# thu-ml/tianshou

Hardware: AMD Instinct MI355X
Metric: PPO learn() update-steps/sec (minibatch 65536, preprocessing incl.) + GAE transitions/sec; cpu_baseline / rocm_eager_baseline are PORTS of the reference path (oracle/), kind=port (higher is better)
Workload: dtype f32; 1 GPU; C2 PPO MuJoCo-shape rollout (BASELINE configs[1]): ONE rollout of 512 envs x 2048 steps = 2^20 transitions, minibatch 65536, obs 17, act 6, MLP[64,64] actor-critic, repeat 10, recompute_advantage off; parallelism=dp1, exchange=none

## Files before the change

include/tsengine.h:

```cpp
#ifndef TSENGINE_H
#define TSENGINE_H

#include <stddef.h>
#include <stdint.h>

#ifdef __cplusplus
extern "C" {
#endif

#define TS_OK 0
#define TS_ERR_INVALID_ARG (-1)
#define TS_ERR_SHAPE (-2)
#define TS_ERR_HIP (-3)
#define TS_ERR_UNSUPPORTED (-4)
#define TS_ERR_WORKSPACE (-5)

typedef void* ts_stream_t;
typedef struct ts_workspace ts_workspace;

const char* ts_version(void);
const char* ts_last_error(void);

int ts_workspace_create(ts_workspace** out, int device, size_t max_bytes);
int ts_workspace_destroy(ts_workspace* ws);
// ... 3 lines not shown
#define TS_KIND_PPO_STEP 0
#define TS_KIND_PPO_REDUCE 1
#define TS_KIND_PPO_ADAM 2
#define TS_KIND_PPO_INFER 3
#define TS_KIND_GAE_MAPS 4
#define TS_KIND_GAE_APPLY 5
#define TS_KIND_CONV_FWD 6
#define TS_KIND_CONV_WGRAD 7
#define TS_KIND_CONV_DGRAD 8
#define TS_N_KINDS 9
int ts_profile_begin(ts_workspace* ws);
int ts_profile_end(ts_workspace* ws, double* h_ms_by_kind, int64_t* h_count_by_kind, int n_kinds);


int64_t ts_gae_num_tiles(int64_t n);
int ts_gae_scan(ts_workspace* ws, const float* v_s, const float* v_s_next, const void* rew,
                int rew_dtype, const uint8_t* terminated, const uint8_t* truncated,
                const int64_t* cut_pos, int64_t n_cut, const int64_t* d_n_cut, int64_t n,
                double gamma, double gae_lambda, double v_scale, double ret_div, float* adv_out,
                float* returns_out, double* adv64, double* ret64, double* ret_partials,
                ts_stream_t stream);

int ts_gae_check(ts_workspace* ws, int* h_error_out, ts_stream_t stream);

int ts_isin_positions(const int64_t* indices, int64_t n, const int64_t* unfinished,
                      int64_t n_unfinished, int64_t* cut_pos_out, int64_t capacity,
                      int64_t* n_cut_out, ts_stream_t stream);

int ts_nstep_return(const double* rew_B, const uint8_t* end_flag_B, const float* target_q_IA,
                    const int64_t* stacked_indices_NI, int64_t I, int64_t A, int64_t n_step,
                    int64_t B, double gamma, float* out, double* out64, ts_stream_t stream);

int ts_nstep_indices(const int64_t* indices, int64_t I, int64_t n_step, const int64_t* offset,
                     int64_t E, const uint8_t* done, const int64_t* last_index,
                     const int64_t* lengths, int64_t* after_out, int64_t* stacked_out,
                     ts_stream_t stream);

int ts_nstep_return_fused(const int64_t* indices, int64_t I, int64_t n_step,
                          const int64_t* offset, int64_t E, const uint8_t* done,
                          const uint8_t* terminated, const int64_t* last_index,
                          const int64_t* lengths, const double* rew_B, const float* target_q_IA,
                          int64_t A, double gamma, float* out, double* out64,
                          ts_stream_t stream);

int ts_nstep_coefficients(const int64_t* indices, int64_t I, int64_t n_step, const int64_t* offset, int64_t E,
                          const uint8_t* done_B, const uint8_t* terminated_B, const int64_t* last_index,
// ... 89 lines not shown
    int32_t optimizer;
    int32_t rms_centered;
    double weight_decay;
    double rms_alpha;
    double rms_momentum;
    double max_action;
} ts_ppo_hparams;
#define TS_OPT_ADAM 0
#define TS_OPT_RMSPROP 1

int ts_ppo_infer(ts_workspace* ws, const float* params, int64_t obs_dim, int64_t act_dim, const float* obs,
                 const float* act, int64_t n, float* v_out, float* logp_out,
                 ts_stream_t stream);
int ts_ppo_infer_bounded(ts_workspace* ws, const float* params, int64_t obs_dim, int64_t act_dim, double max_action,
                         const float* obs, const float* act, int64_t n, float* v_out, float* logp_out, float* mu_out,
                         ts_stream_t stream);

int ts_ppo_update(ts_workspace* ws, float* params, float* adam_m, float* adam_v,
                  int64_t adam_step0, int64_t obs_dim, int64_t act_dim, const float* obs,
                  const float* act, const float* adv, const float* returns,
                  const float* logp_old, const float* v_s, int64_t n, const int64_t* perm,
                  const int64_t* h_mb_offset, int64_t n_steps, const ts_ppo_hparams* hp,
                  float* losses_out, float* grads_out, ts_stream_t stream);

int64_t ts_ppo_record_width(int64_t obs_dim, int64_t act_dim);
int ts_ppo_pack_batch(const float* obs, const float* act, const float* adv, const float* returns,
                      const float* logp_old, const float* v_s, int64_t n, int64_t obs_dim,
                      int64_t act_dim, float* rec_out, ts_stream_t stream);

int ts_ppo_grad(ts_workspace* ws, const float* params, int64_t obs_dim, int64_t act_dim,
                const float* rec, int64_t n, const int64_t* perm_rows, int64_t n_rows,
                int64_t global_batch, const float* adv_stats, const ts_ppo_hparams* hp,
                float* grad_out, float* loss_parts_out, ts_stream_t stream);
int ts_ppo_apply(ts_workspace* ws, float* params, float* adam_m, float* adam_v, int64_t adam_step, int64_t obs_dim,
                 int64_t act_dim, const float* grad, const ts_ppo_hparams* hp, ts_stream_t stream);
int ts_ppo_invalidate_image(ts_workspace* ws);

int ts_ppo_step_plan(int64_t obs_dim, int64_t act_dim, int64_t n_rows, int32_t nets, int32_t* variant_out,
                     int32_t* grid_out, int32_t* slabs_out);


int ts_polyak_update(float* tgt, const float* src, int64_t n, double tau, ts_stream_t stream);

int ts_adam_step(ts_workspace* ws, float* params, float* adam_m, float* adam_v, const float* grad, int64_t n,
                 int64_t step, double lr, double beta1, double beta2, double eps, double max_grad_norm,
                 ts_stream_t stream);
// ... 492 lines not shown
```

tianshou_amd/_lib.py:

```python
from __future__ import annotations

import ctypes as C
import os
import re

_PKG = os.path.dirname(os.path.abspath(__file__))
LIB_PATH = os.environ.get("TS_LIB_PATH") or os.path.join(_PKG, "lib", "libtsengine.so")
HEADER_PATH = os.path.join(os.path.dirname(_PKG), "include", "tsengine.h")

TS_OK = 0
TS_ERR_INVALID_ARG = -1
TS_ERR_SHAPE = -2
TS_ERR_HIP = -3
TS_ERR_UNSUPPORTED = -4
TS_ERR_WORKSPACE = -5


class EngineError(RuntimeError):

    def __init__(self, code: int, msg: str):
        super().__init__(f"libtsengine error {code}: {msg}")
        self.code = code


# ... 130 lines not shown
    @property
    def handle(self) -> C.c_void_p:
        return self._h

    profiling = False

    def profile_begin(self) -> None:
        check(load().ts_profile_begin(self._h))
        self.profiling = True

    def profile_end(self) -> dict[str, tuple[float, int]]:
        n = len(KERNEL_KINDS)
        ms = (C.c_double * n)()
        cnt = (C.c_int64 * n)()
        check(load().ts_profile_end(self._h, ms, cnt, C.c_int(n)))
        self.profiling = False
        return {k: (float(ms[i]), int(cnt[i])) for i, k in enumerate(KERNEL_KINDS)}

    def gae_check(self) -> int:
        err = C.c_int(0)
        check(load().ts_gae_check(self._h, C.byref(err), current_stream()))
        return int(err.value)

    def close(self) -> None:
        if self._h:
            load().ts_workspace_destroy(self._h)
            self._h = C.c_void_p(0)

    def __del__(self):
        try:
            self.close()
        except Exception:
            pass


_default_ws: dict[tuple[int, int], Workspace] = {}


def default_workspace(device_index: int) -> Workspace:
    import torch

    try:
        stream = int(_raw_stream(device_index))
    except Exception:
        stream = 0
    key = (device_index, stream)
# ... 22 lines not shown
```

tianshou_amd/csrc/ts_common.h:

```cpp
#pragma once
#include <hip/hip_runtime.h>

#include <atomic>
#include <cstdarg>
#include <cstdint>
#include <cstdio>

#include "../../include/tsengine.h"

namespace ts {

char* err_buf();
int fail(int code, const char* fmt, ...);

#define TS_HIP_CHECK(expr)                                                                 \
    do {                                                                                   \
        hipError_t _e = (expr);                                                            \
        if (_e != hipSuccess)                                                              \
            return ts::fail(TS_ERR_HIP, "%s failed: %s (%s:%d)", #expr, hipGetErrorString(_e), \
                            __FILE__, __LINE__);                                           \
    } while (0)

#define TS_LAUNCH_CHECK()                                                                  \
    do {                                                                                   \
// ... 26 lines not shown
    unsigned long long gae_ticket_base[8];
    unsigned int gae_epoch;
    int profiling;
    hipEvent_t* ev;
    int* ev_kind;
    int ev_cap, ev_n;
    void* ppo_image;
    size_t ppo_image_bytes;
    const float* ppo_image_params;
    int ppo_image_key;
    void* conv_scratch[2];
    size_t conv_scratch_bytes[2];
    void* dg_tables;
    long long dg_key[16][16];
    int dg_next[2];
    hipStream_t side;
    hipStream_t side2;
    hipEvent_t side_ev[16];
    int side_ready;
    hipEvent_t td_ev;
    int td_ev_ready;
    void* learn_graphs;
    void (*learn_graphs_free)(void*);
};

namespace ts {
int ws_reserve(ts_workspace* ws, size_t bytes);
int ws_winner(ts_workspace* ws, int64_t bound, hipStream_t stream, int32_t** out);

int side_stream(ts_workspace* ws, hipStream_t main, hipStream_t* out);
int stream_wait(ts_workspace* ws, hipStream_t from, hipStream_t to, int slot);
int side_streams(ts_workspace* ws, hipStream_t main, hipStream_t* a, hipStream_t* b);
int record_td(ts_workspace* ws, hipStream_t s);
void adam_step_scalars(int64_t step, double lr, double beta1, double beta2, float out[2]);
int adam_step_dev(hipStream_t s, float* params, float* m, float* v, const float* grad, int64_t n, const float* step_dev,
                  double beta1, double beta2, double eps, double max_grad_norm, float* norm_scratch);
int uniform_fill_f64(double* out, int64_t n, uint64_t seed, uint64_t counter, const uint64_t* counter_dev, hipStream_t s);

struct DynLds {
    std::atomic<int> granted[16] = {};
    int allow(const void* fn, size_t bytes) {
        int dev = 0;
        if (hipGetDevice(&dev) != hipSuccess || dev < 0) dev = 0;
        std::atomic<int>& g = granted[dev & 15];
        if ((int)bytes <= g.load(std::memory_order_acquire)) return TS_OK;
        hipError_t e = hipFuncSetAttribute(fn, hipFuncAttributeMaxDynamicSharedMemorySize, (int)bytes);
// ... 55 lines not shown
```

tianshou_amd/csrc/ts_core.hip:

```cpp
#include <cstdlib>
#include <cstring>

#include "ts_common.h"

namespace ts {

char* err_buf() {
    static thread_local char buf[512] = {0};
    return buf;
}

int fail(int code, const char* fmt, ...) {
    va_list ap;
    va_start(ap, fmt);
    vsnprintf(err_buf(), 512, fmt, ap);
    va_end(ap);
    return code;
}

int ws_reserve(ts_workspace* ws, size_t bytes) {
    if (!ws) return fail(TS_ERR_WORKSPACE, "workspace is NULL");
    if (bytes <= ws->bytes) return TS_OK;
    if (ws->max_bytes && bytes > ws->max_bytes)
        return fail(TS_ERR_WORKSPACE, "workspace needs %zu bytes, limit is %zu", bytes, ws->max_bytes);
// ... 146 lines not shown
    return TS_OK;
}

int ts_workspace_side_stream(ts_workspace* ws, int which, ts_stream_t* stream_out) {
    TS_REQUIRE(ws != nullptr && stream_out != nullptr, TS_ERR_WORKSPACE, "ts_workspace_side_stream: NULL argument");
    TS_REQUIRE(which == 0 || which == 1, TS_ERR_INVALID_ARG, "ts_workspace_side_stream: which = 0 or 1");
    if (int rc = ts::side_create(ws)) return rc;
    *stream_out = reinterpret_cast<ts_stream_t>(which == 0 ? ws->side : ws->side2);
    return TS_OK;
}

int ts_workspace_destroy(ts_workspace* ws) {
    if (!ws) return TS_OK;
    if (ws->learn_graphs && ws->learn_graphs_free) { (void)hipSetDevice(ws->device); ws->learn_graphs_free(ws->learn_graphs); }
    if (ws->side_ready) {
        (void)hipSetDevice(ws->device);
        (void)hipStreamSynchronize(ws->side);
        for (int i = 0; i < 16; ++i) (void)hipEventDestroy(ws->side_ev[i]);
        (void)hipStreamSynchronize(ws->side2);
        (void)hipStreamDestroy(ws->side);
        (void)hipStreamDestroy(ws->side2);
    }
    if (ws->td_ev_ready) { (void)hipSetDevice(ws->device); (void)hipEventDestroy(ws->td_ev); }
    if (ws->ppo_image) { (void)hipSetDevice(ws->device); (void)hipDeviceSynchronize(); (void)hipFree(ws->ppo_image); }
    for (int k = 0; k < 2; ++k)
        if (ws->conv_scratch[k]) { (void)hipSetDevice(ws->device); (void)hipDeviceSynchronize(); (void)hipFree(ws->conv_scratch[k]); }
    if (ws->dg_tables) { (void)hipSetDevice(ws->device); (void)hipDeviceSynchronize(); (void)hipFree(ws->dg_tables); }
    if (ws->base || ws->winner || ws->ev || ws->gae_sync) {
        (void)hipSetDevice(ws->device);
        (void)hipDeviceSynchronize();
        if (ws->gae_sync) (void)hipFree(ws->gae_sync);
        if (ws->base) (void)hipFree(ws->base);
        if (ws->winner) (void)hipFree(ws->winner);
        if (ws->ev) {
            for (int i = 0; i < 2 * ws->ev_cap; ++i) (void)hipEventDestroy(ws->ev[i]);
            free(ws->ev);
            free(ws->ev_kind);
        }
    }
    free(ws);
    return TS_OK;
}

}
```

tianshou_amd/csrc/ts_ppo.hip:

```cpp
#include <cstdlib>

#include "ts_common.h"

namespace {

using f32x16 = __attribute__((ext_vector_type(16))) float;
using f32x4 = __attribute__((ext_vector_type(4))) float;

constexpr int HID = 64;
constexpr int W2_PITCH = 68;
constexpr int W2_SIZE = HID * W2_PITCH;
constexpr int ACT_PAD = 8;
constexpr int TILE_PITCH = 36;
constexpr int TILE_SIZE = 32 * TILE_PITCH;
constexpr int STEP_THREADS = 256;
constexpr int STEP_WAVES = STEP_THREADS / 64;
constexpr int N_EXTRA = 2;

__device__ __forceinline__ int featF(int r, int h) { return (r & 3) + 8 * (r >> 2) + 4 * h; }

__device__ __forceinline__ f32x16 mfma32(float a, float b, f32x16 c) {
    return __builtin_amdgcn_mfma_f32_32x32x2f32(a, b, c, 0, 0, 0);
}

// ... 1128 lines not shown
                                                       const float* __restrict__ ret,
                                                       const float* __restrict__ logp_old,
                                                       const float* __restrict__ v_old, int64_t n,
                                                       int obs_dim, int act_dim, int rec_w,
                                                       float* __restrict__ rec) {
    const int64_t total = n * rec_w;
    const int64_t stride = (int64_t)gridDim.x * blockDim.x;
    for (int64_t t = (int64_t)blockIdx.x * blockDim.x + threadIdx.x; t < total; t += stride) {
        const int64_t row = t / rec_w;
        const int c = (int)(t - row * rec_w);
        float v = 0.f;
        if (c < obs_dim) v = obs[row * obs_dim + c];
        else if (c < obs_dim + act_dim) v = act[row * act_dim + (c - obs_dim)];
        else if (c == obs_dim + act_dim) v = adv[row];
        else if (c == obs_dim + act_dim + 1) v = ret[row];
        else if (c == obs_dim + act_dim + 2) v = logp_old[row];
        else if (c == obs_dim + act_dim + 3) v = v_old[row];
        rec[t] = v;
    }
}

__global__ __launch_bounds__(1024) void ppo_adv_stats_kernel(const float* __restrict__ adv,
                                                             const int64_t* __restrict__ perm,
                                                             const int64_t* __restrict__ mb_offset,
                                                             float* __restrict__ out) {
    __shared__ double r1[16], r2[16];
    const int64_t lo = mb_offset[blockIdx.x], hi = mb_offset[blockIdx.x + 1];
    double s1 = 0.0, s2 = 0.0;
    for (int64_t k = lo + threadIdx.x; k < hi; k += 1024) {
        const double v = (double)adv[perm ? perm[k] : k];
        s1 += v;
        s2 += v * v;
    }
#pragma unroll
    for (int off = 32; off > 0; off >>= 1) {
        s1 += __shfl_down(s1, off, 64);
        s2 += __shfl_down(s2, off, 64);
    }
    if ((threadIdx.x & 63) == 0) { r1[threadIdx.x >> 6] = s1; r2[threadIdx.x >> 6] = s2; }
    __syncthreads();
    if (threadIdx.x == 0) {
        double t1 = 0.0, t2 = 0.0;
        for (int w = 0; w < 16; ++w) { t1 += r1[w]; t2 += r2[w]; }
        const double n = (double)(hi - lo);
        const double mean = t1 / n;
        const double var = (t2 - n * mean * mean) / (n - 1.0);
        out[2 * blockIdx.x] = (float)mean;
        out[2 * blockIdx.x + 1] = (float)sqrt(var > 0.0 ? var : 0.0);
    }
}

template <int KS1>
size_t infer_lds_bytes() { return sizeof(float) * (size_t)Lds<KS1, 2>::END; }
// ... 507 lines not shown
    return rec_width(obs_dim, act_dim);
}

int ts_ppo_pack_batch(const float* obs, const float* act, const float* adv, const float* returns,
                      const float* logp_old, const float* v_s, int64_t n, int64_t obs_dim,
                      int64_t act_dim, float* rec_out, ts_stream_t stream) {
    int rc = check_dims(obs_dim, act_dim);
    if (rc != TS_OK) return rc;
    TS_REQUIRE(n >= 0, TS_ERR_INVALID_ARG, "ts_ppo_pack_batch: negative n");
    if (n == 0) return TS_OK;
    TS_REQUIRE(obs && act && adv && returns && logp_old && v_s && rec_out, TS_ERR_INVALID_ARG,
               "ts_ppo_pack_batch: NULL argument");
    TS_REQUIRE((reinterpret_cast<uintptr_t>(rec_out) & 15u) == 0, TS_ERR_INVALID_ARG,
               "ts_ppo_pack_batch: rec_out must be 16-byte aligned");
    const int rw = rec_width(obs_dim, act_dim);
    int64_t blocks = (n * rw + 255) / 256;
    if (blocks > 8192) blocks = 8192;
    hipLaunchKernelGGL(ppo_pack_kernel, dim3((unsigned)blocks), dim3(256), 0, ts::as_stream(stream), obs, act,
                       adv, returns, logp_old, v_s, n, (int)obs_dim, (int)act_dim, rw, rec_out);
    TS_LAUNCH_CHECK();
    return TS_OK;
}

int ts_ppo_update(ts_workspace* ws, float* params, float* adam_m, float* adam_v,
                  int64_t adam_step0, int64_t obs_dim, int64_t act_dim, const float* obs,
                  const float* act, const float* adv, const float* returns,
                  const float* logp_old, const float* v_s, int64_t n, const int64_t* perm,
                  const int64_t* h_mb_offset, int64_t n_steps, const ts_ppo_hparams* hp,
                  float* losses_out, float* grads_out, ts_stream_t stream) {
    int rc = check_dims(obs_dim, act_dim);
    if (rc != TS_OK) return rc;
    TS_REQUIRE(n >= 1 && n_steps >= 0 && adam_step0 >= 0, TS_ERR_INVALID_ARG, "ts_ppo_update: bad size");
    if (n_steps == 0) return TS_OK;
    TS_REQUIRE(ws && params && adam_m && adam_v && obs && act && adv && returns && logp_old && v_s &&
                   h_mb_offset && hp,
               TS_ERR_INVALID_ARG, "ts_ppo_update: NULL argument");
    const Dims d = make_dims((int)obs_dim, (int)act_dim);
    const int ks = supported_ks(ks1_for((int)obs_dim));
    size_t slab_floats = 0;
    int slab_w = 0;
    int64_t last_rows = -1;
    for (int64_t k = 0; k < n_steps; ++k) {
        const int64_t rows = h_mb_offset[k + 1] - h_mb_offset[k];
        TS_REQUIRE(rows >= 1, TS_ERR_SHAPE, "ts_ppo_update: minibatch %lld is empty", (long long)k);
        TS_REQUIRE(perm || h_mb_offset[k + 1] <= n, TS_ERR_SHAPE, "ts_ppo_update: minibatch beyond n");
        if (rows == last_rows) continue;
        last_rows = rows;
        const StepPlan pl = plan_step(d, ks, rows, hp->nets, hp->max_action > 0.0);
        slab_floats = std::max(slab_floats, (size_t)pl.n_slabs * (size_t)pl.slab_w);
        slab_w = std::max(slab_w, pl.slab_w);
    }
    const int rw = rec_width(obs_dim, act_dim);
    const WsLayout wl = ws_layout((int)((slab_floats + slab_w - 1) / slab_w), slab_w, n_steps);
    const size_t off_bytes = (sizeof(int64_t) * (size_t)(n_steps + 1) + 255) & ~(size_t)255;
    const size_t rec_bytes = (sizeof(float) * (size_t)n * rw + 255) & ~(size_t)255;
    const ImageBuf ib = image_buf(d, ks);
    const size_t img_bytes = ib.img_bytes, inv_bytes = ib.inv_bytes;
    const int img_end = ib.img_end;
    rc = ts::ws_reserve(ws, wl.total + off_bytes + rec_bytes + img_bytes + inv_bytes + 256);
    if (rc != TS_OK) return rc;
    char* base = reinterpret_cast<char*>(ws->base);
    float* image = reinterpret_cast<float*>(base + wl.total + off_bytes + rec_bytes);
    int* inv = reinterpret_cast<int*>(base + wl.total + off_bytes + rec_bytes + img_bytes);
    float* slabs = reinterpret_cast<float*>(base + wl.slabs);
    float* grad = reinterpret_cast<float*>(base + wl.grad);
    float* sumsq = reinterpret_cast<float*>(base + wl.sumsq);
    float* advstats = reinterpret_cast<float*>(base + wl.advstats);
    int64_t* d_off = reinterpret_cast<int64_t*>(base + wl.total);
    float* rec = reinterpret_cast<float*>(base + wl.total + off_bytes);
    hipStream_t s = ts::as_stream(stream);

    rc = ts_ppo_pack_batch(obs, act, adv, returns, logp_old, v_s, n, obs_dim, act_dim, rec, stream);
    if (rc != TS_OK) return rc;
    rc = build_image(s, params, d, ks, image, inv);
    if (rc != TS_OK) return rc;
    if (hp->adv_norm) {
        TS_HIP_CHECK(hipMemcpyAsync(d_off, h_mb_offset, sizeof(int64_t) * (size_t)(n_steps + 1),
                                    hipMemcpyHostToDevice, s));
        hipLaunchKernelGGL(ppo_adv_stats_kernel, dim3((unsigned)n_steps), dim3(1024), 0, s, adv, perm,
                           d_off, advstats);
        TS_LAUNCH_CHECK();
    }
    for (int64_t k = 0; k < n_steps; ++k) {
        StepArgs g{};
        g.params = params;
        g.rec_w = rw;
        g.n_rows = h_mb_offset[k + 1] - h_mb_offset[k];
        if (perm) { g.rec = rec; g.rows = perm + h_mb_offset[k]; }
        else { g.rec = rec + h_mb_offset[k] * rw; g.rows = nullptr; }
        g.inv_batch = 1.0f / (float)g.n_rows;
        g.adv_stats = hp->adv_norm ? advstats + 2 * k : nullptr;
        g.image = image;
        fill_hparams(g, hp);
        float* losses = losses_out ? losses_out + 4 * k : nullptr;
        const StepPlan pl = plan_step(d, ks, g.n_rows, hp->nets, hp->max_action > 0.0);
        rc = run_grad(ws, g, d, ks, pl, slabs, grad, sumsq, losses, s);
        if (rc != TS_OK) return rc;
        AdamArgs a = adam_args(params, adam_m, adam_v, adam_step0 + k + 1, d, hp);
        a.grad = grad; a.sumsq_part = sumsq; a.n_part = (pl.slab_w + 63) / 64;
        a.losses = losses; a.apply = 1;
        a.image = image; a.inv = inv; a.sig_off = d.a_sig; a.act = d.act; a.small0 = img_end - 32;
        if (grads_out && k == n_steps - 1)
            TS_HIP_CHECK(hipMemcpyAsync(grads_out, grad, sizeof(float) * (size_t)d.p_total,
                                        hipMemcpyDeviceToDevice, s));
        {
            ts::ProfScope prof(ws, TS_KIND_PPO_ADAM, s);
            hipLaunchKernelGGL(ppo_adam_kernel, dim3((d.p_total + ADAM_THREADS - 1) / ADAM_THREADS),
                               dim3(ADAM_THREADS), 0, s, a);
        }
        TS_LAUNCH_CHECK();
    }
    return TS_OK;
}

int ts_ppo_grad(ts_workspace* ws, const float* params, int64_t obs_dim, int64_t act_dim,
                const float* rec, int64_t n, const int64_t* perm_rows, int64_t n_rows,
                int64_t global_batch, const float* adv_stats, const ts_ppo_hparams* hp,
                float* grad_out, float* loss_parts_out, ts_stream_t stream) {
    int rc = check_dims(obs_dim, act_dim);
    if (rc != TS_OK) return rc;
    TS_REQUIRE(n_rows >= 1 && global_batch >= n_rows, TS_ERR_SHAPE, "ts_ppo_grad: bad batch sizes");
    TS_REQUIRE(ws && params && rec && hp && grad_out, TS_ERR_INVALID_ARG, "ts_ppo_grad: NULL argument");
    TS_REQUIRE(perm_rows || n_rows <= n, TS_ERR_SHAPE, "ts_ppo_grad: n_rows > n");
    TS_REQUIRE(!hp->adv_norm || adv_stats, TS_ERR_INVALID_ARG, "ts_ppo_grad: adv_norm needs adv_stats");
    TS_REQUIRE((reinterpret_cast<uintptr_t>(rec) & 15u) == 0, TS_ERR_INVALID_ARG,
               "ts_ppo_grad: rec must be 16-byte aligned");
    const Dims d = make_dims((int)obs_dim, (int)act_dim);
    const int ks = supported_ks(ks1_for((int)obs_dim));
    const StepPlan pl = plan_step(d, ks, n_rows, hp->nets, hp->max_action > 0.0);
    const WsLayout wl = ws_layout(pl.n_slabs, pl.slab_w, 1);
    rc = ts::ws_reserve(ws, wl.total);
    if (rc != TS_OK) return rc;
    char* base = reinterpret_cast<char*>(ws->base);
    hipStream_t s = ts::as_stream(stream);
    float* image; int* inv;
// ... 128 lines not shown
```

tianshou_amd/csrc/ts_returns.hip:

```cpp
#include <algorithm>
#include <cstdlib>

#include "ts_common.h"

#pragma clang fp contract(off)

namespace {

constexpr int GAE_THREADS = 256;
constexpr int GAE_ITEMS = 8;
constexpr int GAE_TILE = GAE_THREADS * GAE_ITEMS;
constexpr int GAE_WAVES = GAE_THREADS / 64;

struct Aff {
    double a, b;
};

__device__ __forceinline__ Aff aff_identity() { return Aff{1.0, 0.0}; }

__device__ __forceinline__ Aff compose(const Aff& L, const Aff& R) {
    return Aff{L.a * R.a, L.b + L.a * R.b};
}

__device__ __forceinline__ Aff shfl_down_aff(const Aff& v, int off) {
// ... 656 lines not shown
    hipStream_t s = ts::as_stream(stream);
    if (rew_dtype == 0) {
        GaeArgs<float> g{v_s, v_s_next, (const float*)rew, terminated, truncated, cut_pos, d_n_cut,
                         n_cut, n, gamma, gamma * gae_lambda, v_scale, ret_div};
        return launch_gae(ws, g, adv_out, returns_out, adv64, ret64, ret_partials, s);
    }
    GaeArgs<double> g{v_s, v_s_next, (const double*)rew, terminated, truncated, cut_pos, d_n_cut,
                      n_cut, n, gamma, gamma * gae_lambda, v_scale, ret_div};
    return launch_gae(ws, g, adv_out, returns_out, adv64, ret64, ret_partials, s);
}

int ts_gae_check(ts_workspace* ws, int* error_out, ts_stream_t stream) {
    TS_REQUIRE(ws && error_out, TS_ERR_INVALID_ARG, "ts_gae_check: NULL argument");
    *error_out = 0;
    if (!ws->gae_sync) return TS_OK;
    GaeSyncHeader h;
    hipStream_t s = ts::as_stream(stream);
    TS_HIP_CHECK(hipMemcpyAsync(&h, ws->gae_sync, sizeof(h), hipMemcpyDeviceToHost, s));
    TS_HIP_CHECK(hipStreamSynchronize(s));
    *error_out = (int)h.error;
    return TS_OK;
}

int ts_isin_positions(const int64_t* indices, int64_t n, const int64_t* unfinished,
                      int64_t n_unfinished, int64_t* cut_pos_out, int64_t capacity,
                      int64_t* n_cut_out, ts_stream_t stream) {
    TS_REQUIRE(n >= 0 && n_unfinished >= 0 && capacity >= 0, TS_ERR_INVALID_ARG,
               "ts_isin_positions: negative size");
    TS_REQUIRE(n_cut_out, TS_ERR_INVALID_ARG, "ts_isin_positions: n_cut_out is NULL");
    hipStream_t s = ts::as_stream(stream);
    TS_HIP_CHECK(hipMemsetAsync(n_cut_out, 0, sizeof(int64_t), s));
    if (n == 0 || n_unfinished == 0) return TS_OK;
    TS_REQUIRE(indices && unfinished && cut_pos_out, TS_ERR_INVALID_ARG,
               "ts_isin_positions: NULL array argument");
    hipLaunchKernelGGL(isin_positions_kernel, dim3(grid_for(n, 256)), dim3(256), 0, s, indices, n,
                       unfinished, n_unfinished, cut_pos_out, capacity,
                       reinterpret_cast<unsigned long long*>(n_cut_out));
    TS_LAUNCH_CHECK();
    return TS_OK;
}

int ts_nstep_return(const double* rew_B, const uint8_t* end_flag_B, const float* target_q_IA,
                    const int64_t* stacked_indices_NI, int64_t I, int64_t A, int64_t n_step,
                    int64_t B, double gamma, float* out, double* out64, ts_stream_t stream) {
    TS_REQUIRE(I >= 0 && A >= 0 && B >= 0, TS_ERR_INVALID_ARG, "ts_nstep_return: negative size");
    TS_REQUIRE(n_step >= 1, TS_ERR_INVALID_ARG, "ts_nstep_return: n_step must be >= 1");
// ... 66 lines not shown
```

tianshou_amd/ppo.py:

```python
from __future__ import annotations

import ctypes as C
import math
from dataclasses import dataclass

import numpy as np
import torch

from . import _lib
from .buffer import _dev_index
from .returns import gae_scan

HIDDEN = 64
PARAM_ORDER = ("a_w1", "a_b1", "a_w2", "a_b2", "a_wmu", "a_bmu", "a_sigma",
               "c_w1", "c_b1", "c_w2", "c_b2", "c_wv", "c_bv")


def param_shapes(obs_dim: int, act_dim: int) -> dict[str, tuple[int, ...]]:
    return {
        "a_w1": (HIDDEN, obs_dim), "a_b1": (HIDDEN,), "a_w2": (HIDDEN, HIDDEN), "a_b2": (HIDDEN,),
        "a_wmu": (act_dim, HIDDEN), "a_bmu": (act_dim,), "a_sigma": (act_dim,),
        "c_w1": (HIDDEN, obs_dim), "c_b1": (HIDDEN,), "c_w2": (HIDDEN, HIDDEN), "c_b2": (HIDDEN,),
        "c_wv": (1, HIDDEN), "c_bv": (1,),
    }
# ... 139 lines not shown
    w = int(lib.ts_ppo_record_width(_lib.i64(obs_dim), _lib.i64(act_dim)))
    rec = torch.empty((n, w), dtype=torch.float32, device=b["obs"].device)
    _lib.check(lib.ts_ppo_pack_batch(
        _lib.ptr(b["obs"]), _lib.ptr(b["act"]), _lib.ptr(b["adv"]), _lib.ptr(b["returns"]),
        _lib.ptr(b["logp_old"]), _lib.ptr(b["v_s"]), _lib.i64(n), _lib.i64(obs_dim), _lib.i64(act_dim),
        _lib.ptr(rec), _lib.current_stream(rec.device)))
    return rec


class PPOEngine:

    def __init__(self, obs_dim: int, act_dim: int, flat_params: torch.Tensor, cfg: PPOConfig):
        if not flat_params.is_cuda:
            raise RuntimeError("PPOEngine needs its parameters on an MI355X; there is no CPU fallback")
        self.obs_dim, self.act_dim, self.cfg = obs_dim, act_dim, cfg
        self.P = param_count(obs_dim, act_dim)
        if flat_params.numel() != self.P:
            raise ValueError(f"flat_params has {flat_params.numel()} entries, layout needs {self.P}")
        self.params = flat_params.detach().to(torch.float32).contiguous().clone()
        self.adam_m = torch.zeros_like(self.params)
        self.adam_v = torch.zeros_like(self.params)
        self.adam_step = 0
        self.device = self.params.device
        self.ret_rms = [0.0, 1.0, 0.0]
        self._eps = 1e-8
        self._ws = _lib.default_workspace(_dev_index(self.params))

    def check(self) -> None:
        if self._ws.gae_check():
            raise _lib.EngineError(-1, "gae_single_pass: a tile hand-off timed out; advantages / returns are invalid")

    def _f32(self, x) -> torch.Tensor:
        if not isinstance(x, torch.Tensor):
            x = torch.as_tensor(np.asarray(x), device=self.device)
        return x.to(device=self.device, dtype=torch.float32).contiguous()

    def add_returns_and_advantages(self, obs, obs_next, rew, terminated, truncated, cut_pos,
                                   d_n_cut=None, reduce_stats=None, v_s=None):
        cfg = self.cfg
        if v_s is None:
            v_s, _ = infer(self.params, self.obs_dim, self.act_dim, obs)
        v_next, _ = infer(self.params, self.obs_dim, self.act_dim, obs_next)
        scale = math.sqrt(self.ret_rms[1] + self._eps) if cfg.return_scaling else 1.0
        out = gae_scan(v_s, v_next, rew, terminated, truncated, cut_pos, gamma=cfg.gamma,
                       gae_lambda=cfg.gae_lambda, v_scale=scale, ret_div=scale,
                       want_ret_stats=cfg.return_scaling, d_n_cut=d_n_cut, ws=self._ws)
        if cfg.return_scaling:
            n = float(v_s.numel())
            s1, s2 = float(out["ret_sum"]), float(out["ret_sumsq"])
            if reduce_stats is not None:
                s1, s2, n = reduce_stats(s1, s2, n)
            self.ret_rms = rms_merge(self.ret_rms, s1, s2, n)
        return v_s, out["returns"], out["adv"]

    def preprocess(self, obs, obs_next, act, rew, terminated, truncated, cut_pos, d_n_cut=None, reduce_stats=None):
        obs, obs_next, act = self._f32(obs), self._f32(obs_next), self._f32(act)
        if self.cfg.algo == "a2c":
            v_s, returns, adv = self.add_returns_and_advantages(obs, obs_next, rew, terminated,
                                                                truncated, cut_pos, d_n_cut, reduce_stats)
            logp_old = torch.zeros_like(adv)
        else:
            v_s0, logp_old = infer(self.params, self.obs_dim, self.act_dim, obs, act, want_v=True, want_logp=True,
                                   max_action=self.cfg.max_action)
            v_s, returns, adv = self.add_returns_and_advantages(obs, obs_next, rew, terminated, truncated, cut_pos,
                                                                d_n_cut, reduce_stats, v_s=v_s0)
        return {"obs": obs, "obs_next": obs_next, "act": act, "rew": rew, "terminated": terminated,
                "truncated": truncated, "cut_pos": cut_pos, "d_n_cut": d_n_cut,
                "v_s": v_s, "returns": returns, "adv": adv, "logp_old": logp_old}

    def _run_steps(self, b: dict, perm: torch.Tensor | None, offsets: list[int], want_grad=False):
        n_steps = len(offsets) - 1
        losses = torch.empty((n_steps, 4), dtype=torch.float32, device=self.device)
        grads = torch.empty(self.P, dtype=torch.float32, device=self.device) if want_grad else None
        h_off = (C.c_int64 * len(offsets))(*offsets)
        hp = self.cfg.to_c()
        _lib.check(_lib.load().ts_ppo_update(
            self._ws.handle, _lib.ptr(self.params), _lib.ptr(self.adam_m), _lib.ptr(self.adam_v),
            _lib.i64(self.adam_step), _lib.i64(self.obs_dim), _lib.i64(self.act_dim),
            _lib.ptr(b["obs"]), _lib.ptr(b["act"]), _lib.ptr(b["adv"]), _lib.ptr(b["returns"]),
            _lib.ptr(b["logp_old"]), _lib.ptr(b["v_s"]), _lib.i64(b["obs"].shape[0]), _lib.ptr(perm),
            h_off, _lib.i64(n_steps), C.byref(hp), _lib.ptr(losses), _lib.ptr(grads),
            _lib.current_stream(self.device)))
        self.adam_step += n_steps
        return losses, grads

    def update(self, b: dict, batch_size: int | None, repeat: int, perms=None, want_grad=False):
        n = b["obs"].shape[0]
        cfg = self.cfg
        if perms is None:
            perms = [np.random.permutation(n) for _ in range(repeat)]
        offs1 = split_offsets(n, batch_size, merge_last=True)
        out, grads = [], None
        if not cfg.recompute_advantage:
            if all(isinstance(p, torch.Tensor) for p in perms):
                perm = torch.cat([p.to(device=self.device, dtype=torch.int64) for p in perms])
            else:
                perm = torch.as_tensor(np.concatenate([np.asarray(p, dtype=np.int64) for p in perms]),
                                       device=self.device)
            offsets = [r * n + o for r in range(repeat) for o in offs1[:-1]] + [repeat * n]
            losses, grads = self._run_steps(b, perm, offsets, want_grad)
            out.append(losses)
        else:
            for r in range(repeat):
                if r > 0:
                    v_s, returns, adv = self.add_returns_and_advantages(
                        b["obs"], b["obs_next"], b["rew"], b["terminated"], b["truncated"],
                        b["cut_pos"], b.get("d_n_cut"))
                    b = dict(b, v_s=v_s, returns=returns, adv=adv)
                perm = (perms[r].to(device=self.device, dtype=torch.int64) if isinstance(perms[r], torch.Tensor)
                        else torch.as_tensor(np.asarray(perms[r], dtype=np.int64), device=self.device))
                losses, grads = self._run_steps(b, perm, offs1, want_grad)
                out.append(losses)
        losses = torch.cat(out, dim=0)
        steps = losses.shape[0]
        return (losses, steps, grads) if want_grad else (losses, steps)


def summary_stats(seq: np.ndarray) -> dict[str, float]:
    seq = np.asarray(seq, dtype=np.float64)
    return {"mean": float(seq.mean()), "std": float(seq.std()), "max": float(seq.max()),
            "min": float(seq.min())}
```

tianshou_amd/returns.py:

```python
from __future__ import annotations

import numpy as np
import torch

from . import _lib
from .buffer import DeviceReplayBuffer, _dev_index, _i64_dev, _u8_dev


def _f32(x, device) -> torch.Tensor:
    if isinstance(x, torch.Tensor):
        return x.to(device=device, dtype=torch.float32).reshape(-1).contiguous()
    return torch.as_tensor(np.asarray(x, dtype=np.float32).reshape(-1), device=device)


def gae_scan(v_s, v_s_next, rew, terminated, truncated, cut_pos=None, *, gamma=0.99,
             gae_lambda=0.95, v_scale=1.0, ret_div=1.0, want_f64=False, want_ret_stats=False,
             d_n_cut=None, ws=None):
    dev = v_s.device
    v_s = _f32(v_s, dev)
    v_s_next = _f32(v_s_next, dev)
    n = v_s.numel()
    if isinstance(rew, torch.Tensor):
        rew = rew.to(dev).reshape(-1)
        if rew.dtype not in (torch.float32, torch.float64):
# ... 10 lines not shown
        n_cut = cut_pos.numel()
    adv = torch.empty(n, dtype=torch.float32, device=dev)
    ret = torch.empty(n, dtype=torch.float32, device=dev)
    adv64 = torch.empty(n, dtype=torch.float64, device=dev) if want_f64 else None
    ret64 = torch.empty(n, dtype=torch.float64, device=dev) if want_f64 else None
    lib = _lib.load()
    parts = None
    if want_ret_stats:
        parts = torch.zeros(2 * max(int(lib.ts_gae_num_tiles(n)), 1), dtype=torch.float64, device=dev)
    if ws is None:
        ws = _lib.default_workspace(_dev_index(v_s))
    _lib.check(lib.ts_gae_scan(
        ws.handle, _lib.ptr(v_s), _lib.ptr(v_s_next), _lib.ptr(rew),
        0 if rew.dtype == torch.float32 else 1, _lib.ptr(terminated), _lib.ptr(truncated),
        _lib.ptr(cut_pos), _lib.i64(n_cut), _lib.ptr(d_n_cut), _lib.i64(n), _lib.f64(gamma),
        _lib.f64(gae_lambda), _lib.f64(v_scale), _lib.f64(ret_div), _lib.ptr(adv), _lib.ptr(ret),
        _lib.ptr(adv64), _lib.ptr(ret64), _lib.ptr(parts), _lib.current_stream(dev)))
    out = {"adv": adv, "returns": ret}
    if want_f64:
        out["adv64"], out["ret64"] = adv64, ret64
    if want_ret_stats:
        p = parts.view(-1, 2).sum(dim=0)
        out["ret_sum"], out["ret_sumsq"] = p[0], p[1]
    return out


def _gae(v_s, v_s_, rew, end_flag, gamma: float, gae_lambda: float) -> torch.Tensor:
    dev = v_s.device if isinstance(v_s, torch.Tensor) else torch.device("cuda")
    end = _u8_dev(end_flag, dev)
    zeros = torch.zeros_like(end)
    return gae_scan(_f32(v_s, dev), _f32(v_s_, dev), rew, zeros, end, gamma=gamma,
                    gae_lambda=gae_lambda, want_f64=True)["adv64"]


def cut_positions(buffer: DeviceReplayBuffer, indices: torch.Tensor):
    dev = buffer.device
    unf, n_unf = buffer._unfinished_raw()
    indices = _i64_dev(indices, dev).reshape(-1)
    pad = torch.full_like(unf, torch.iinfo(torch.int64).max)
    ar = torch.arange(unf.numel(), device=dev)
    unf_sorted = torch.where(ar < n_unf, unf, pad)
    cut = torch.empty(max(unf.numel(), 1), dtype=torch.int64, device=dev)
    d_n = torch.zeros(1, dtype=torch.int64, device=dev)
    _lib.check(_lib.load().ts_isin_positions(
        _lib.ptr(indices), _lib.i64(indices.numel()), _lib.ptr(unf_sorted), _lib.i64(unf.numel()),
        _lib.ptr(cut), _lib.i64(cut.numel()), _lib.ptr(d_n), _lib.current_stream(dev)))
# ... 112 lines not shown
```

Before: 15620 update-steps/s.

## Pass per-repeat permutation table and defer return-stat readback asynchronously

PPO learn no longer concatenates the per-repeat permutation tensors. It passes a host table of permutation pointers to a new update entry point, which maps each minibatch to its repeat's permutation and offset, including inside the advantage-stats kernel. Return-scaling statistics are also no longer synchronously read back as Python floats during preprocessing. They are copied asynchronously into pinned host memory behind an event and resolved lazily when ret_rms is read. This removes a large device concat and a blocking host sync per learn call, at the cost of extra validation, a lazy-state property, and stream-lifetime bookkeeping for the permutation tensors.

```diff
diff --git a/include/tsengine.h b/include/tsengine.h
--- a/include/tsengine.h
+++ b/include/tsengine.h
@@ -49,6 +49,9 @@
                 ts_stream_t stream);
 
 int ts_gae_check(ts_workspace* ws, int* h_error_out, ts_stream_t stream);
+
+int ts_ret_stats_enqueue(ts_workspace* ws, const double* d_sums, uint64_t* seq_out, ts_stream_t stream);
+int ts_ret_stats_wait(ts_workspace* ws, uint64_t seq, double* h_sum_out, double* h_sumsq_out);
 
 int ts_isin_positions(const int64_t* indices, int64_t n, const int64_t* unfinished,
                       int64_t n_unfinished, int64_t* cut_pos_out, int64_t capacity,
@@ -184,6 +187,12 @@
                   const float* logp_old, const float* v_s, int64_t n, const int64_t* perm,
                   const int64_t* h_mb_offset, int64_t n_steps, const ts_ppo_hparams* hp,
                   float* losses_out, float* grads_out, ts_stream_t stream);
+int ts_ppo_update_perms(ts_workspace* ws, float* params, float* adam_m, float* adam_v,
+                        int64_t adam_step0, int64_t obs_dim, int64_t act_dim, const float* obs,
+                        const float* act, const float* adv, const float* returns,
+                        const float* logp_old, const float* v_s, int64_t n, const int64_t* const* perms,
+                        int64_t n_perms, int64_t rows_per_perm, const int64_t* h_mb_offset, int64_t n_steps,
+                        const ts_ppo_hparams* hp, float* losses_out, float* grads_out, ts_stream_t stream);
 
 int64_t ts_ppo_record_width(int64_t obs_dim, int64_t act_dim);
 int ts_ppo_pack_batch(const float* obs, const float* act, const float* adv, const float* returns,
diff --git a/tianshou_amd/_lib.py b/tianshou_amd/_lib.py
--- a/tianshou_amd/_lib.py
+++ b/tianshou_amd/_lib.py
@@ -176,6 +176,28 @@
         check(load().ts_gae_check(self._h, C.byref(err), current_stream()))
         return int(err.value)
 
+    _stats_owner = None
+
+    def ret_stats_enqueue(self, sums, owner) -> int:
+        import weakref
+
+        self.ret_stats_collect()
+        seq = C.c_uint64(0)
+        check(load().ts_ret_stats_enqueue(self._h, ptr(sums), C.byref(seq), current_stream(sums.device)))
+        self._stats_owner = weakref.ref(owner)
+        return int(seq.value)
+
+    def ret_stats_collect(self) -> None:
+        ref, self._stats_owner = self._stats_owner, None
+        owner = ref() if ref is not None else None
+        if owner is not None:
+            owner._resolve_ret_stats()
+
+    def ret_stats_wait(self, seq: int) -> tuple[float, float]:
+        s1, s2 = C.c_double(0.0), C.c_double(0.0)
+        check(load().ts_ret_stats_wait(self._h, C.c_uint64(seq), C.byref(s1), C.byref(s2)))
+        return float(s1.value), float(s2.value)
+
     def close(self) -> None:
         if self._h:
             load().ts_workspace_destroy(self._h)
diff --git a/tianshou_amd/csrc/ts_common.h b/tianshou_amd/csrc/ts_common.h
--- a/tianshou_amd/csrc/ts_common.h
+++ b/tianshou_amd/csrc/ts_common.h
@@ -72,6 +72,11 @@
     int td_ev_ready;
     void* learn_graphs;
     void (*learn_graphs_free)(void*);
+    void* ret_slot;
+    hipEvent_t ret_ev;
+    int ret_ready;
+    int ret_inflight;
+    unsigned long long ret_seq;
 };
 
 namespace ts {
diff --git a/tianshou_amd/csrc/ts_core.hip b/tianshou_amd/csrc/ts_core.hip
--- a/tianshou_amd/csrc/ts_core.hip
+++ b/tianshou_amd/csrc/ts_core.hip
@@ -192,6 +192,12 @@
         (void)hipStreamDestroy(ws->side2);
     }
     if (ws->td_ev_ready) { (void)hipSetDevice(ws->device); (void)hipEventDestroy(ws->td_ev); }
+    if (ws->ret_ready) {
+        (void)hipSetDevice(ws->device);
+        if (ws->ret_inflight) (void)hipEventSynchronize(ws->ret_ev);
+        (void)hipEventDestroy(ws->ret_ev);
+        (void)hipHostFree(ws->ret_slot);
+    }
     if (ws->ppo_image) { (void)hipSetDevice(ws->device); (void)hipDeviceSynchronize(); (void)hipFree(ws->ppo_image); }
     for (int k = 0; k < 2; ++k)
         if (ws->conv_scratch[k]) { (void)hipSetDevice(ws->device); (void)hipDeviceSynchronize(); (void)hipFree(ws->conv_scratch[k]); }
diff --git a/tianshou_amd/csrc/ts_ppo.hip b/tianshou_amd/csrc/ts_ppo.hip
--- a/tianshou_amd/csrc/ts_ppo.hip
+++ b/tianshou_amd/csrc/ts_ppo.hip
@@ -1174,13 +1174,21 @@
 
 __global__ __launch_bounds__(1024) void ppo_adv_stats_kernel(const float* __restrict__ adv,
                                                              const int64_t* __restrict__ perm,
+                                                             const int64_t* const* __restrict__ perm_tab,
+                                                             int64_t rows_per_perm,
                                                              const int64_t* __restrict__ mb_offset,
                                                              float* __restrict__ out) {
     __shared__ double r1[16], r2[16];
     const int64_t lo = mb_offset[blockIdx.x], hi = mb_offset[blockIdx.x + 1];
+    int64_t shift = 0;
+    if (perm_tab) {
+        const int64_t r = lo / rows_per_perm;
+        perm = perm_tab[r];
+        shift = r * rows_per_perm;
+    }
     double s1 = 0.0, s2 = 0.0;
     for (int64_t k = lo + threadIdx.x; k < hi; k += 1024) {
-        const double v = (double)adv[perm ? perm[k] : k];
+        const double v = (double)adv[perm ? perm[k - shift] : k];
         s1 += v;
         s2 += v * v;
     }
@@ -1734,12 +1742,13 @@
     return TS_OK;
 }
 
-int ts_ppo_update(ts_workspace* ws, float* params, float* adam_m, float* adam_v,
-                  int64_t adam_step0, int64_t obs_dim, int64_t act_dim, const float* obs,
-                  const float* act, const float* adv, const float* returns,
-                  const float* logp_old, const float* v_s, int64_t n, const int64_t* perm,
-                  const int64_t* h_mb_offset, int64_t n_steps, const ts_ppo_hparams* hp,
-                  float* losses_out, float* grads_out, ts_stream_t stream) {
+static int ppo_update_impl(ts_workspace* ws, float* params, float* adam_m, float* adam_v,
+                           int64_t adam_step0, int64_t obs_dim, int64_t act_dim, const float* obs,
+                           const float* act, const float* adv, const float* returns,
+                           const float* logp_old, const float* v_s, int64_t n, const int64_t* perm,
+                           const int64_t* const* perms, int64_t n_perms, int64_t rows_per_perm,
+                           const int64_t* h_mb_offset, int64_t n_steps, const ts_ppo_hparams* hp,
+                           float* losses_out, float* grads_out, ts_stream_t stream) {
     int rc = check_dims(obs_dim, act_dim);
     if (rc != TS_OK) return rc;
     TS_REQUIRE(n >= 1 && n_steps >= 0 && adam_step0 >= 0, TS_ERR_INVALID_ARG, "ts_ppo_update: bad size");
@@ -1747,6 +1756,20 @@
     TS_REQUIRE(ws && params && adam_m && adam_v && obs && act && adv && returns && logp_old && v_s &&
                    h_mb_offset && hp,
                TS_ERR_INVALID_ARG, "ts_ppo_update: NULL argument");
+    if (perms) {
+        TS_REQUIRE(n_perms >= 1 && rows_per_perm >= 1, TS_ERR_INVALID_ARG, "ts_ppo_update_perms: bad permutation table size");
+        for (int64_t r = 0; r < n_perms; ++r)
+            TS_REQUIRE(perms[r], TS_ERR_INVALID_ARG, "ts_ppo_update_perms: permutation %lld is NULL", (long long)r);
+        for (int64_t k = 0; k < n_steps; ++k) {
+            const int64_t lo = h_mb_offset[k], hi = h_mb_offset[k + 1];
+            TS_REQUIRE(lo >= 0 && lo / rows_per_perm < n_perms, TS_ERR_SHAPE,
+                       "ts_ppo_update_perms: minibatch %lld starts outside the %lld permutations", (long long)k, (long long)n_perms);
+            TS_REQUIRE(hi <= (lo / rows_per_perm + 1) * rows_per_perm, TS_ERR_SHAPE,
+                       "ts_ppo_update_perms: minibatch %lld crosses a repeat boundary", (long long)k);
+        }
+    } else {
+        n_perms = 0;
+    }
     const Dims d = make_dims((int)obs_dim, (int)act_dim);
     const int ks = supported_ks(ks1_for((int)obs_dim));
     size_t slab_floats = 0;
@@ -1755,7 +1778,7 @@
     for (int64_t k = 0; k < n_steps; ++k) {
         const int64_t rows = h_mb_offset[k + 1] - h_mb_offset[k];
         TS_REQUIRE(rows >= 1, TS_ERR_SHAPE, "ts_ppo_update: minibatch %lld is empty", (long long)k);
-        TS_REQUIRE(perm || h_mb_offset[k + 1] <= n, TS_ERR_SHAPE, "ts_ppo_update: minibatch beyond n");
+        TS_REQUIRE(perm || perms || h_mb_offset[k + 1] <= n, TS_ERR_SHAPE, "ts_ppo_update: minibatch beyond n");
         if (rows == last_rows) continue;
         last_rows = rows;
         const StepPlan pl = plan_step(d, ks, rows, hp->nets, hp->max_action > 0.0);
@@ -1764,7 +1787,7 @@
     }
     const int rw = rec_width(obs_dim, act_dim);
     const WsLayout wl = ws_layout((int)((slab_floats + slab_w - 1) / slab_w), slab_w, n_steps);
-    const size_t off_bytes = (sizeof(int64_t) * (size_t)(n_steps + 1) + 255) & ~(size_t)255;
+    const size_t off_bytes = (sizeof(int64_t) * (size_t)(n_steps + 1 + n_perms) + 255) & ~(size_t)255;
     const size_t rec_bytes = (sizeof(float) * (size_t)n * rw + 255) & ~(size_t)255;
     const ImageBuf ib = image_buf(d, ks);
     const size_t img_bytes = ib.img_bytes, inv_bytes = ib.inv_bytes;
@@ -1789,8 +1812,15 @@
     if (hp->adv_norm) {
         TS_HIP_CHECK(hipMemcpyAsync(d_off, h_mb_offset, sizeof(int64_t) * (size_t)(n_steps + 1),
                                     hipMemcpyHostToDevice, s));
-        hipLaunchKernelGGL(ppo_adv_stats_kernel, dim3((unsigned)n_steps), dim3(1024), 0, s, adv, perm,
-                           d_off, advstats);
+        const int64_t* const* d_tab = nullptr;
+        if (perms) {
+            static_assert(sizeof(const int64_t*) == sizeof(int64_t), "the pointer table shares the offsets' area");
+            TS_HIP_CHECK(hipMemcpyAsync(d_off + n_steps + 1, perms, sizeof(const int64_t*) * (size_t)n_perms,
+                                        hipMemcpyHostToDevice, s));
+            d_tab = reinterpret_cast<const int64_t* const*>(d_off + n_steps + 1);
+        }
+        hipLaunchKernelGGL(ppo_adv_stats_kernel, dim3((unsigned)n_steps), dim3(1024), 0, s, adv, perm, d_tab,
+                           rows_per_perm, d_off, advstats);
         TS_LAUNCH_CHECK();
     }
     for (int64_t k = 0; k < n_steps; ++k) {
@@ -1798,7 +1828,11 @@
         g.params = params;
         g.rec_w = rw;
         g.n_rows = h_mb_offset[k + 1] - h_mb_offset[k];
-        if (perm) { g.rec = rec; g.rows = perm + h_mb_offset[k]; }
+        if (perms) {
+            const int64_t r = h_mb_offset[k] / rows_per_perm;
+            g.rec = rec; g.rows = perms[r] + (h_mb_offset[k] - r * rows_per_perm);
+        }
+        else if (perm) { g.rec = rec; g.rows = perm + h_mb_offset[k]; }
         else { g.rec = rec + h_mb_offset[k] * rw; g.rows = nullptr; }
         g.inv_batch = 1.0f / (float)g.n_rows;
         g.adv_stats = hp->adv_norm ? advstats + 2 * k : nullptr;
@@ -1823,6 +1857,27 @@
         TS_LAUNCH_CHECK();
     }
     return TS_OK;
+}
+
+int ts_ppo_update(ts_workspace* ws, float* params, float* adam_m, float* adam_v,
+                  int64_t adam_step0, int64_t obs_dim, int64_t act_dim, const float* obs,
+                  const float* act, const float* adv, const float* returns,
+                  const float* logp_old, const float* v_s, int64_t n, const int64_t* perm,
+                  const int64_t* h_mb_offset, int64_t n_steps, const ts_ppo_hparams* hp,
+                  float* losses_out, float* grads_out, ts_stream_t stream) {
+    return ppo_update_impl(ws, params, adam_m, adam_v, adam_step0, obs_dim, act_dim, obs, act, adv, returns, logp_old, v_s,
+                           n, perm, nullptr, 0, 0, h_mb_offset, n_steps, hp, losses_out, grads_out, stream);
+}
+
+int ts_ppo_update_perms(ts_workspace* ws, float* params, float* adam_m, float* adam_v,
+                        int64_t adam_step0, int64_t obs_dim, int64_t act_dim, const float* obs,
+                        const float* act, const float* adv, const float* returns,
+                        const float* logp_old, const float* v_s, int64_t n, const int64_t* const* perms,
+                        int64_t n_perms, int64_t rows_per_perm, const int64_t* h_mb_offset, int64_t n_steps,
+                        const ts_ppo_hparams* hp, float* losses_out, float* grads_out, ts_stream_t stream) {
+    TS_REQUIRE(perms, TS_ERR_INVALID_ARG, "ts_ppo_update_perms: perms is NULL");
+    return ppo_update_impl(ws, params, adam_m, adam_v, adam_step0, obs_dim, act_dim, obs, act, adv, returns, logp_old, v_s,
+                           n, nullptr, perms, n_perms, rows_per_perm, h_mb_offset, n_steps, hp, losses_out, grads_out, stream);
 }
 
 int ts_ppo_grad(ts_workspace* ws, const float* params, int64_t obs_dim, int64_t act_dim,
diff --git a/tianshou_amd/csrc/ts_returns.hip b/tianshou_amd/csrc/ts_returns.hip
--- a/tianshou_amd/csrc/ts_returns.hip
+++ b/tianshou_amd/csrc/ts_returns.hip
@@ -702,6 +702,48 @@
     return TS_OK;
 }
 
+struct RetSlot {
+    double sum, sumsq;
+    unsigned long long seq;
+};
+
+int ts_ret_stats_enqueue(ts_workspace* ws, const double* d_sums, uint64_t* seq_out, ts_stream_t stream) {
+    TS_REQUIRE(ws && d_sums && seq_out, TS_ERR_INVALID_ARG, "ts_ret_stats_enqueue: NULL argument");
+    if (!ws->ret_ready) {
+        TS_HIP_CHECK(hipSetDevice(ws->device));
+        TS_HIP_CHECK(hipHostMalloc(&ws->ret_slot, sizeof(RetSlot), hipHostMallocDefault));
+        if (hipEventCreateWithFlags(&ws->ret_ev, hipEventDisableTiming) != hipSuccess) {
+            (void)hipHostFree(ws->ret_slot);
+            ws->ret_slot = nullptr;
+            return ts::fail(TS_ERR_HIP, "ts_ret_stats_enqueue: hipEventCreateWithFlags failed");
+        }
+        ws->ret_ready = 1;
+    }
+    if (ws->ret_inflight) TS_HIP_CHECK(hipEventSynchronize(ws->ret_ev));
+    RetSlot* slot = reinterpret_cast<RetSlot*>(ws->ret_slot);
+    hipStream_t s = ts::as_stream(stream);
+    slot->seq = ++ws->ret_seq;
+    ws->ret_inflight = 0;
+    TS_HIP_CHECK(hipMemcpyAsync(slot, d_sums, 2 * sizeof(double), hipMemcpyDeviceToHost, s));
+    TS_HIP_CHECK(hipEventRecord(ws->ret_ev, s));
+    ws->ret_inflight = 1;
+    *seq_out = slot->seq;
+    return TS_OK;
+}
+
+int ts_ret_stats_wait(ts_workspace* ws, uint64_t seq, double* h_sum_out, double* h_sumsq_out) {
+    TS_REQUIRE(ws && h_sum_out && h_sumsq_out, TS_ERR_INVALID_ARG, "ts_ret_stats_wait: NULL argument");
+    TS_REQUIRE(ws->ret_ready && ws->ret_inflight, TS_ERR_WORKSPACE, "ts_ret_stats_wait: no read-back is pending");
+    const volatile RetSlot* slot = reinterpret_cast<const volatile RetSlot*>(ws->ret_slot);
+    TS_REQUIRE(slot->seq == seq, TS_ERR_WORKSPACE, "ts_ret_stats_wait: read-back %llu was overwritten by %llu",
+               (unsigned long long)seq, slot->seq);
+    TS_HIP_CHECK(hipEventSynchronize(ws->ret_ev));
+    *h_sum_out = slot->sum;
+    *h_sumsq_out = slot->sumsq;
+    ws->ret_inflight = 0;
+    return TS_OK;
+}
+
 int ts_isin_positions(const int64_t* indices, int64_t n, const int64_t* unfinished,
                       int64_t n_unfinished, int64_t* cut_pos_out, int64_t capacity,
                       int64_t* n_cut_out, ts_stream_t stream) {
diff --git a/tianshou_amd/ppo.py b/tianshou_amd/ppo.py
--- a/tianshou_amd/ppo.py
+++ b/tianshou_amd/ppo.py
@@ -185,9 +185,29 @@
         self.adam_v = torch.zeros_like(self.params)
         self.adam_step = 0
         self.device = self.params.device
-        self.ret_rms = [0.0, 1.0, 0.0]
+        self._ret_rms = [0.0, 1.0, 0.0]
+        self._rms_pending = None
         self._eps = 1e-8
         self._ws = _lib.default_workspace(_dev_index(self.params))
+
+    @property
+    def ret_rms(self) -> list:
+        if self._rms_pending is not None:
+            self._resolve_ret_stats()
+        return self._ret_rms
+
+    @ret_rms.setter
+    def ret_rms(self, value) -> None:
+        self._rms_pending = None
+        self._ret_rms = list(value)
+
+    def _resolve_ret_stats(self) -> None:
+        pending, self._rms_pending = self._rms_pending, None
+        if pending is None:
+            return
+        n, seq, _sums = pending
+        s1, s2 = self._ws.ret_stats_wait(seq)
+        self._ret_rms = rms_merge(self._ret_rms, s1, s2, n)
 
     def check(self) -> None:
         if self._ws.gae_check():
@@ -210,10 +230,13 @@
                        want_ret_stats=cfg.return_scaling, d_n_cut=d_n_cut, ws=self._ws)
         if cfg.return_scaling:
             n = float(v_s.numel())
-            s1, s2 = float(out["ret_sum"]), float(out["ret_sumsq"])
-            if reduce_stats is not None:
+            if reduce_stats is None:
+                seq = self._ws.ret_stats_enqueue(out["ret_sums"], self)
+                self._rms_pending = (n, seq, out["ret_sums"])
+            else:
+                s1, s2 = float(out["ret_sum"]), float(out["ret_sumsq"])
                 s1, s2, n = reduce_stats(s1, s2, n)
-            self.ret_rms = rms_merge(self.ret_rms, s1, s2, n)
+                self.ret_rms = rms_merge(self.ret_rms, s1, s2, n)
         return v_s, out["returns"], out["adv"]
 
     def preprocess(self, obs, obs_next, act, rew, terminated, truncated, cut_pos, d_n_cut=None, reduce_stats=None):
@@ -231,19 +254,32 @@
                 "truncated": truncated, "cut_pos": cut_pos, "d_n_cut": d_n_cut,
                 "v_s": v_s, "returns": returns, "adv": adv, "logp_old": logp_old}
 
-    def _run_steps(self, b: dict, perm: torch.Tensor | None, offsets: list[int], want_grad=False):
+    def _run_steps(self, b: dict, perm, offsets: list[int], want_grad=False):
         n_steps = len(offsets) - 1
         losses = torch.empty((n_steps, 4), dtype=torch.float32, device=self.device)
         grads = torch.empty(self.P, dtype=torch.float32, device=self.device) if want_grad else None
         h_off = (C.c_int64 * len(offsets))(*offsets)
         hp = self.cfg.to_c()
-        _lib.check(_lib.load().ts_ppo_update(
-            self._ws.handle, _lib.ptr(self.params), _lib.ptr(self.adam_m), _lib.ptr(self.adam_v),
-            _lib.i64(self.adam_step), _lib.i64(self.obs_dim), _lib.i64(self.act_dim),
-            _lib.ptr(b["obs"]), _lib.ptr(b["act"]), _lib.ptr(b["adv"]), _lib.ptr(b["returns"]),
-            _lib.ptr(b["logp_old"]), _lib.ptr(b["v_s"]), _lib.i64(b["obs"].shape[0]), _lib.ptr(perm),
-            h_off, _lib.i64(n_steps), C.byref(hp), _lib.ptr(losses), _lib.ptr(grads),
-            _lib.current_stream(self.device)))
+        if isinstance(perm, (list, tuple)):
+            tab = (C.c_void_p * len(perm))(*[_lib.ptr(p) for p in perm])
+            _lib.check(_lib.load().ts_ppo_update_perms(
+                self._ws.handle, _lib.ptr(self.params), _lib.ptr(self.adam_m), _lib.ptr(self.adam_v),
+                _lib.i64(self.adam_step), _lib.i64(self.obs_dim), _lib.i64(self.act_dim),
+                _lib.ptr(b["obs"]), _lib.ptr(b["act"]), _lib.ptr(b["adv"]), _lib.ptr(b["returns"]),
+                _lib.ptr(b["logp_old"]), _lib.ptr(b["v_s"]), _lib.i64(b["obs"].shape[0]), tab,
+                _lib.i64(len(perm)), _lib.i64(perm[0].numel()), h_off, _lib.i64(n_steps), C.byref(hp), _lib.ptr(losses),
+                _lib.ptr(grads), _lib.current_stream(self.device)))
+            stream = torch.cuda.current_stream(self.device)
+            for p in perm:
+                p.record_stream(stream)
+        else:
+            _lib.check(_lib.load().ts_ppo_update(
+                self._ws.handle, _lib.ptr(self.params), _lib.ptr(self.adam_m), _lib.ptr(self.adam_v),
+                _lib.i64(self.adam_step), _lib.i64(self.obs_dim), _lib.i64(self.act_dim),
+                _lib.ptr(b["obs"]), _lib.ptr(b["act"]), _lib.ptr(b["adv"]), _lib.ptr(b["returns"]),
+                _lib.ptr(b["logp_old"]), _lib.ptr(b["v_s"]), _lib.i64(b["obs"].shape[0]), _lib.ptr(perm),
+                h_off, _lib.i64(n_steps), C.byref(hp), _lib.ptr(losses), _lib.ptr(grads),
+                _lib.current_stream(self.device)))
         self.adam_step += n_steps
         return losses, grads
 
@@ -255,7 +291,11 @@
         offs1 = split_offsets(n, batch_size, merge_last=True)
         out, grads = [], None
         if not cfg.recompute_advantage:
-            if all(isinstance(p, torch.Tensor) for p in perms):
+            if repeat >= 1 and len(perms) == repeat and all(
+                    isinstance(p, torch.Tensor) and p.dtype == torch.int64 and p.device == self.device
+                    and p.dim() == 1 and p.numel() == n and p.is_contiguous() for p in perms):
+                perm = list(perms)
+            elif all(isinstance(p, torch.Tensor) for p in perms):
                 perm = torch.cat([p.to(device=self.device, dtype=torch.int64) for p in perms])
             else:
                 perm = torch.as_tensor(np.concatenate([np.asarray(p, dtype=np.int64) for p in perms]),
@@ -274,7 +314,7 @@
                         else torch.as_tensor(np.asarray(perms[r], dtype=np.int64), device=self.device))
                 losses, grads = self._run_steps(b, perm, offs1, want_grad)
                 out.append(losses)
-        losses = torch.cat(out, dim=0)
+        losses = out[0] if len(out) == 1 else torch.cat(out, dim=0)
         steps = losses.shape[0]
         return (losses, steps, grads) if want_grad else (losses, steps)
 
diff --git a/tianshou_amd/returns.py b/tianshou_amd/returns.py
--- a/tianshou_amd/returns.py
+++ b/tianshou_amd/returns.py
@@ -56,6 +56,7 @@
     if want_ret_stats:
         p = parts.view(-1, 2).sum(dim=0)
         out["ret_sum"], out["ret_sumsq"] = p[0], p[1]
+        out["ret_sums"] = p
     return out
 
 
```

Measured after the change: 15650 update-steps/s, median of 6. Within noise of the previous version (+0.2%).
